# jamesdolezal/biscuit

Hardware: AMD Instinct MI355X
Metric: tiles/sec at MC-dropout=30, 299x299x3 (Xception, slide-level pred/sigma reduce) (higher is better)
Workload: dtype f16; 1 GPU; BASELINE.json config 2: 1000 synthetic 299x299x3 tiles/slide, Xception f16 storage + MFMA, fp32 accumulation / BN / MC head, MC=30, batch=256, 17664 tiles/GPU resident in HBM; f16 is the 16-bit mode that holds the 1e-3 tile/slide tolerance on O(1)-logit weights (bf16, the type config 2 names, runs 5-6 % slower and misses it: bf16_value); mc_mode=head, mc_n=30, batch=256, hip_streams=2, grids_sized_for_mask=False, parallelism=slide-sharded dp1, one all-gather of slide (pred, sigma, n)

## Files before the change

biscuit_amd/csrc/biscuit_hip.hip:

```cpp
#include "bq_ctx.h"

#include <math.h>
#include <cmath>
#include <stdlib.h>
#include <string.h>

namespace {

std::string g_create_error;

constexpr int pad16(int c) { return (c + 15) / 16 * 16; }

enum LayerFlags : int {
    F_RES = 1,
    F_DWTMP = 2,
    F_SPLIT_TMP = 4,
    F_POOLED = 8
};

struct Layer {
    const char* name;
    const char* out_name;
    int cin, cout;
    int ldi, ldo;
// ... 236 lines not shown

#define TAP_AT(name, buf, H, C, ld) \
    do { int _t = tap_nhwc(w, name, buf, H, C, ld); if (_t) return _t < 0 ? _t : BQ_OK; } while (0)
#define TAP(name, li, buf) TAP_AT(name, buf, kLayers[li].H, kLayers[li].cout, kLayers[li].ldo)

GemmParams gemm_params(const bq_ctx* c, int li, int n, const void* in, const void* residual, void* out) {
    const Layer& L = kLayers[li];
    const GemmLayer& G = c->layers[li];
    GemmParams p{};
    p.in = in; p.wp = G.wp; p.dw = G.dw; p.scale = G.scale; p.bias = G.bias; p.residual = residual; p.out = out;
    p.M = n * L.H * L.H;
    p.K = L.kpad; p.KBtot = L.kpad / (is16(c->cfg.dtype) ? 16 : 8); p.kb0 = 0; p.k_off = 0;
    p.NFp = G.nfp; p.Nstore = L.ldo; p.ldo = L.ldo; p.ldi = L.ldi;
    p.H = L.H; p.W = L.H; p.Hi = L.Hi; p.Wi = L.Hi; p.relu = L.relu;
    return p;
}

struct ConvBufs {
    const void* in; void* out;
    const void* residual = nullptr;
    void* split_tmp = nullptr;
    void* dwtmp = nullptr;
    float* gap_out = nullptr;
};

int launch_conv(const Walk& w, int li, const Route& rt, const ConvBufs& b) {
    bq_ctx* c = w.c;
    const Layer& L = kLayers[li];
    const GemmLayer& G = c->layers[li];
    if (w.plan) { w.note(L.prod == PROD_S2 ? L.out_name : L.name, route_text(rt)); return BQ_OK; }
    const int dtype = c->cfg.dtype, n = w.n, vec = is16(dtype) ? 8 : 4;
    hipStream_t s = w.s;
    const void* residual = (L.flags & F_RES) ? b.residual : nullptr;
    void* dwtmp = (L.flags & F_DWTMP) ? b.dwtmp : nullptr;
    void* split_tmp = (L.flags & F_SPLIT_TMP) ? b.split_tmp : nullptr;
    GemmParams p = gemm_params(c, li, n, b.in, residual, b.out);
    const double es = (double)esize(c);
    const double M = (double)p.M;
    const bool dwp = L.prod == PROD_DW || L.prod == PROD_DW_RELU;
    const double flops = 2.0 * M * L.cin * L.cout + (dwp ? 18.0 * M * L.cin : 0.0);
    const double in_rows = (double)n * L.Hi * L.Hi;
    const double kin = L.prod == PROD_IM2COL ? (double)L.ldi : (double)L.cin;
    const double bytes = es * (in_rows * kin * (L.prod == PROD_S2 ? 0.25 : 1.0) + M * L.cout * (residual ? 2.0 : 1.0)) +
                         es * (double)L.cin * L.cout;
    char cls[96];
    snprintf(cls, sizeof cls, "%s_k%d_n%d_%dx%d",
             L.prod == PROD_S2 ? "res1x1s2" : (L.prod == PROD_IM2COL ? "conv3x3" : "sepconv"), L.cin, L.cout, L.H, L.H);
    const bool two = rt.conv == R_DW_THEN_EXIT;
    ProfScope ps(c, s, two ? std::string("split_") + cls : std::string(cls), two ? 0.0 : flops, two ? 0.0 : bytes);
    const char* what = "launch ";
    int e = 0;
    switch (rt.conv) {
    case R_STREAM:
        what = "launch(stream) ";
        e = launch_sepconv_stream(dtype, L.kpad, L.cout, L.prod == PROD_DW_RELU, b.in, G.wp16, G.dw, G.scale, G.bias, b.out, n, L.H, L.H,
                                  L.relu, c->num_cus, s);
        break;
    case R_TILE:
        what = "launch(tile) ";
        e = launch_tile_conv(dtype, b.in, G.wp, G.scale, G.bias, b.out, n, L.H, L.H, L.Hi, L.Hi, L.relu, c->num_cus, s);
        break;
    case R_DW_THEN_EXIT: {
        const bool gap = rt.gap;
        {
            ProfScope pd(c, s, std::string("dw3x3_") + cls, 18.0 * M * L.cin, 2.0 * es * M * L.cin);
            what = "launch(dw3x3) ";
            e = launch_dw3x3(dtype, b.in, G.dw, dwtmp, n, L.H, L.H, L.ldi, L.prod == PROD_DW_RELU, s);
        }
        if (e) break;
        ProfScope pg(c, s, std::string(gap ? "gemm_gap_" : "gemm_") + cls, 2.0 * M * L.cin * L.cout + (gap ? M * L.cout : 0.0),
                     gap ? es * M * L.cin + 4.0 * n * L.cout : es * (M * L.cin + M * L.cout * (residual ? 2.0 : 1.0)));
        what = "launch(exit_gemm) ";
        e = launch_exit_gemm(dtype, dwtmp, G.wp16, G.scale, G.bias, b.out, gap ? b.gap_out : nullptr, n, L.H * L.H, L.kpad, L.cout, L.relu,
                             c->feat_mul, s);
        break;
    }
    case R_S2_TILED_GEMM:
        what = "launch(gemm_tile s2) ";
        e = launch_gemm_tile(dtype, p, s, false);
        break;
    case R_WIDE:
        what = "launch(wide) ";
        e = launch_sepconv_wide(dtype, L.prod, p, G.wp16, c->num_cus, s);
        break;
    case R_FUSED_GEMM:
        for (int sp = 0; sp < rt.nsplit && e == 0; ++sp) {
            const bool last = sp == rt.nsplit - 1;
            p.K = L.kpad / rt.nsplit;
            p.k_off = sp * p.K;
            p.kb0 = sp * (p.K / (2 * vec));
            p.bias = last ? G.bias : nullptr;
            p.relu = last ? L.relu : 0;
            p.residual = last ? (rt.nsplit > 1 ? split_tmp : residual) : (sp > 0 ? split_tmp : nullptr);
            p.out = last ? b.out : split_tmp;
            e = launch_gemm(dtype, L.prod, rt.shape, p, s);
        }
        break;
// ... 7 lines not shown
    Route rt;
    RUN(route_for(w, li, false, &rt));
    if (gap) *gap = rt.gap;
    return launch_conv(w, li, rt, b);
}

int launch_front_route(const Walk& w, const uint8_t* u8, void* out) {
    bq_ctx* c = w.c;
    const int n = w.n;
    const GemmLayer& G = c->layers[kConv2];
    if (w.plan) { w.note(kLayers[kConv2].name, kRouteNames[R_FRONT]); return BQ_OK; }
    {
        ProfScope ps(c, w.s, "stage_stats", 2.0 * n * kStaged, (double)n * kStaged);
        if (launch_stage_stats(u8, n, 299, c->d_stage_stats, w.s)) return fail(c, BQ_ERR_HIP, "stage stats launch failed");
    }
    const double p1 = (double)n * 149 * 149, p2 = (double)n * 147 * 147;
    ProfScope ps(c, w.s, "front_stage_stem_conv2", 2.0 * p1 * 27 * 32 + 2.0 * p2 * 288 * 64 + 4.0 * n * kStaged,
                 (double)n * kStaged + (double)esize(c) * p2 * 64);
    const int e = launch_front(c->cfg.dtype, u8, reinterpret_cast<const unsigned long long*>(c->d_stage_stats), c->front_ws16, c->stem_s,
                               c->stem_b, c->front_wc16, G.scale, G.bias, out, n, c->num_cus, w.s);
    return e ? launch_failed(c, "launch(front)", "", e) : BQ_OK;
}

int launch_block_end(const Walk& w, int li, const Route& rt, const void* x, const void* y, void* out) {
    bq_ctx* c = w.c;
    const Layer& L = kLayers[li];
    const GemmLayer& G = c->layers[li];
    const GemmLayer& G2 = c->layers[li - 1];
    const int dtype = c->cfg.dtype, n = w.n, ci = L.ldi, co = L.ldo;
    hipStream_t s = w.s;
    const double es = (double)esize(c), M = (double)n * L.Hi * L.Hi, Mo = (double)n * L.H * L.H;
    if (rt.kind == R_CONV_THEN_POOL) {
        RUN(launch_conv(w, li, rt, {x, out}));
        TAP(L.name, li, out);
        if (w.plan) return BQ_OK;
        char cls[64];
        snprintf(cls, sizeof cls, "maxpool_add_%d_c%d", L.Hi, L.cout);
        ProfScope ps(c, s, cls, 9.0 * Mo * co, es * ((double)n * L.Hi * L.Hi * co + 2.0 * Mo * co));
        if (launch_pool_add(y, out, out, n, L.Hi, L.Hi, co, dtype, s)) return fail(c, BQ_ERR_HIP, "pool_add launch failed");
        return BQ_OK;
    }
    if (w.plan) { w.note(L.out_name, route_text(rt)); return BQ_OK; }
    if (rt.kind == R_BLOCK_TAIL) {
        char cls[64];
        snprintf(cls, sizeof cls, "blocktail_%d_c%d", L.Hi, L.cout);
        ProfScope ps(c, s, cls, 2.0 * M * co * co + 18.0 * M * co + 2.0 * Mo * ci * co + 9.0 * Mo * co,
                     es * (M * co + Mo * ci + Mo * co) + es * ((double)co * co + (double)ci * co));
        const int e = launch_block_tail(dtype, co, co, ci, y, G2.wp16, G2.dw, G2.scale, G2.bias, x, G.wp16, G.scale, G.bias, out, n,
                                        L.Hi, L.Hi, c->num_cus, s);
        return e ? launch_failed(c, "launch(block tail) ", kLayers[li - 1].name, e) : BQ_OK;
    }
    ProfScope ps(c, s, std::string("respool_") + std::to_string(L.Hi) + "_c" + std::to_string(L.cout),
                 2.0 * Mo * L.cin * L.cout + 9.0 * Mo * co, es * ((double)n * L.Hi * L.Hi * co + Mo * co + Mo * ci) + es * (double)L.cin * L.cout);
    const int e = launch_gemm_tile(dtype, gemm_params(c, li, n, x, y, out), s, true);
    return e ? launch_failed(c, "launch(gemm_tile pool) ", L.name, e) : BQ_OK;
}

int strided_block(const Walk& w, int s1, const void* x, void* t1, void* t2, void* out) {
    RUN(run_conv(w, s1, {x, t1}));
    TAP(kLayers[s1].name, s1, t1);
    Route end;
    RUN(route_for(w, s1 + 2, false, &end));
    if (end.kind != R_BLOCK_TAIL) {
        RUN(run_conv(w, s1 + 1, {t1, t2}));
        TAP(kLayers[s1 + 1].name, s1 + 1, t2);
    }
    RUN(launch_block_end(w, s1 + 2, end, x, end.kind == R_BLOCK_TAIL ? t1 : t2, out));
    if (w.tapped()) return BQ_OK;
    TAP(kLayers[s1 + 2].out_name, s1 + 2, out);
    return BQ_OK;
}

int backbone_impl(const Walk& w, const void* in_nchw, float* feat, unsigned char* ws, const uint8_t* u8 = nullptr) {
    bq_ctx* c = w.c;
    const int n = w.n, dt = c->cfg.dtype;
    hipStream_t s = w.s;
    const WsLayout L = ws_layout(c, n, 1);
    auto at = [&](size_t off) { return reinterpret_cast<void*>(reinterpret_cast<uintptr_t>(ws) + off); };
    void* A = at(L.a); void* B = at(L.b); void* C = at(L.c); void* R = at(L.r);
    const double es = (double)esize(c);
    Route front;
    RUN(route_for(w, kConv2, u8 != nullptr, &front));
    if (front.kind == R_FRONT) {
        RUN(launch_front_route(w, u8, B));
    } else {
        if (u8) {
            in_nchw = at(L.staged);
            if (!w.plan) RUN(bq_stage(c, u8, n, at(L.staged), (bq_stream_t)s));
        }
        if (wants(w.want(), "staged")) {
// ... 8 lines not shown
            ProfScope ps(c, s, "stem_conv1_3x3s2", 2.0 * px * 27 * 32, es * ((double)n * kStaged + px * 32));
            if (launch_stem1(in_nchw, n, c->stem_w, c->stem_s, c->stem_b, A, dt, s)) return fail(c, BQ_ERR_HIP, "stem1 launch failed");
        }
        TAP_AT("block1_conv1", A, 149, 32, 32);
        RUN(launch_conv(w, kConv2, front, {A, B}));
    }
    TAP(kLayers[kConv2].name, kConv2, B);
    void* X = B; void* Y = R;
    for (int s1 = kBlock2; s1 < kBlock5; s1 += 3) {
        RUN(strided_block(w, s1, X, A, C, Y));
        if (w.tapped()) return BQ_OK;
        void* t = X; X = Y; Y = t;
    }
    void* S = B; Y = A;
    for (int s1 = kBlock5; s1 < kBlock13; s1 += 3) {
        RUN(run_conv(w, s1, {X, Y, nullptr, nullptr, S}));
        TAP(kLayers[s1].name, s1, Y);
        RUN(run_conv(w, s1 + 1, {Y, C, nullptr, nullptr, S}));
        TAP(kLayers[s1 + 1].name, s1 + 1, C);
        RUN(run_conv(w, s1 + 2, {C, Y, X, nullptr, S}));
        void* t = X; X = Y; Y = t;
        TAP(kLayers[s1 + 2].out_name, s1 + 2, X);
    }
    RUN(strided_block(w, kBlock13, X, Y, C, S));
    if (w.tapped()) return BQ_OK;
    RUN(run_conv(w, kBlock14, {S, Y, nullptr, C, X}));
    TAP(kLayers[kBlock14].name, kBlock14, Y);
    bool pooled = false;
    RUN(run_conv(w, kBlock14 + 1, {Y, C, nullptr, S, X, feat}, &pooled));
    if (!pooled) {
        TAP(kLayers[kBlock14 + 1].name, kBlock14 + 1, C);
        if (w.plan) {
            w.note("global_avg_pool", "GAP_KERNEL");
        } else {
            ProfScope ps(c, s, "global_avg_pool", (double)n * 100 * 2048, es * (double)n * 100 * 2048 + 4.0 * n * 2048);
            if (launch_gap(C, n, 100, 2048, 2048, feat, c->feat_mul, dt, s)) return fail(c, BQ_ERR_HIP, "gap launch failed");
        }
    }
    if (w.want()) return fail(c, BQ_ERR_ARG, std::string("unknown activation: ") + w.want());
    return BQ_OK;
}

int head_impl(bq_ctx* c, const float* feat, int n, int64_t tile0, int mc_n, int pass0, uint64_t seed,
              int init, int finalize, float* state, float* mean2, float* std2, unsigned char* ws,
              hipStream_t s) {
    const WsLayout L = ws_layout(c, n, mc_n);
    float* h0 = (float*)(ws + L.h0);
    float* h1 = (float*)(ws + L.h1);
    float* rmax = (float*)(ws + L.rmax);
    const unsigned thresh = c->drop_thresh;
    const float dscale = c->drop_scale;
    const int rows = n * mc_n;
// ... 218 lines not shown
            if (we->second.n < 4) return fail(c, BQ_ERR_WEIGHTS, "bad size for " + name + "/wexp");
            memcpy(&wexp, hb + (we->second.p - c->d_blob), 4);
            if (wexp < -64 || wexp > 64) return fail(c, BQ_ERR_WEIGHTS, name + "/wexp must lie in [-64, 64]");
        }
        c->head[layer] = HeadLayer{wh->second.p, wl->second.p, reinterpret_cast<const float*>(bi->second.p), K, wexp};
    }
    c->loaded = true;
    return BQ_OK;
}

int bq_stream_create_masked(bq_ctx* c, const uint32_t* cu_mask, int mask_words, bq_stream_t* out) {
    if (!c || !cu_mask || mask_words <= 0 || !out) return fail(c, BQ_ERR_ARG, "bq_stream_create_masked: bad argument");
    hipStream_t s = nullptr;
    DeviceGuard guard(c->device);
    if (!guard.ok) return fail(c, BQ_ERR_HIP, "hipSetDevice failed");
    HIPCHK(c, hipExtStreamCreateWithCUMask(&s, (uint32_t)mask_words, cu_mask));
    *out = (bq_stream_t)s;
    return BQ_OK;
}

int bq_set_option(bq_ctx* c, const char* name, int value) {
    if (!c || !name) return fail(c, BQ_ERR_ARG, "bq_set_option: bad argument");
    if (strcmp(name, "inflate_variant") == 0 && (value == 0 || value == 5)) { c->inflate_variant = value; return BQ_OK; }
    return fail(c, BQ_ERR_ARG, std::string("bq_set_option: unknown option or value: ") + name);
}

int bq_set_num_cus(bq_ctx* c, int n) {
    if (!c || n < 0 || n > 1024) return fail(c, BQ_ERR_ARG, "bq_set_num_cus: bad argument");
    int dev_cus = 256;
    if (n == 0) {
        hipDeviceProp_t prop;
        if (hipGetDeviceProperties(&prop, c->device) == hipSuccess && prop.multiProcessorCount > 0) dev_cus = prop.multiProcessorCount;
    }
    c->num_cus = n > 0 ? n : dev_cus;
    return BQ_OK;
}

int bq_stream_destroy(bq_ctx* c, bq_stream_t stream) {
    if (!c || !stream) return fail(c, BQ_ERR_ARG, "bq_stream_destroy: bad argument");
    HIPCHK(c, hipStreamDestroy((hipStream_t)stream));
    return BQ_OK;
}

int bq_backbone(bq_ctx* c, const void* d_in, int n, float* d_feat, void* d_ws, size_t ws_bytes,
                bq_stream_t stream) {
    if (!c || !d_in || !d_feat || !d_ws || n <= 0 || n > c->cfg.max_batch) return fail(c, BQ_ERR_ARG, "bq_backbone: bad argument");
// ... 128 lines not shown
```

biscuit_amd/csrc/bq_common.h:

```cpp
#pragma once
#include <hip/hip_runtime.h>
#include <stdint.h>
#include <stddef.h>


struct BqLdsAttr {
    static constexpr int kMaxDev = 64;
    size_t set[kMaxDev] = {};
    int ensure(const void* kern, size_t lds) {
        int dev = -1;
        if (hipGetDevice(&dev) != hipSuccess || dev < 0 || dev >= kMaxDev) dev = -1;
        if (dev >= 0 && lds <= set[dev]) return 0;
        const hipError_t e = hipFuncSetAttribute(kern, hipFuncAttributeMaxDynamicSharedMemorySize, (int)lds);
        if (e != hipSuccess) return (int)e;
        if (dev >= 0) set[dev] = lds;
        return 0;
    }
};

typedef __bf16 bf16_t;
typedef __bf16 bf16x8 __attribute__((ext_vector_type(8)));
typedef _Float16 f16_t;
typedef _Float16 f16x8 __attribute__((ext_vector_type(8)));
typedef float f32x16 __attribute__((ext_vector_type(16)));
// ... 35 lines not shown
    int Nstore;
    int ldo;
    int ldi;
    int H, W;
    int Hi, Wi;
    int relu;
    int unused[2];
};

size_t gemm_lds_bytes(int dtype, int shape, int K);
int launch_gemm(int dtype, int prod, int shape, const GemmParams& p, hipStream_t s);
int gemm_tile_rows(int shape);
bool wide_supported(int dtype, int prod, int nfp, int H, int W, int K, int Nstore, int ldi, int ldo, long long M, bool residual);
int launch_sepconv_wide(int dtype, int prod, const GemmParams& p, const void* wp16, int num_cus, hipStream_t s);
bool stream_supported(int dtype, int cin, int cout, bool relu_in, long long n, int H, int W);
int launch_sepconv_stream(int dtype, int cin, int cout, bool relu_in, const void* in, const void* wp16, const float* dw,
                          const float* scale, const float* bias, void* out, int n, int H, int W, int relu, int num_cus,
                          hipStream_t s);
bool tail_supported(int dtype, int cin, int cout, int cx, long long n, int H, int W);
int launch_block_tail(int dtype, int cin, int cout, int cx, const void* y1, const void* wp16, const float* dw,
                      const float* scale, const float* bias, const void* x, const void* wr16, const float* rscale,
                      const float* rbias, void* out, int n, int H, int W, int num_cus, hipStream_t s);
int launch_dw3x3(int dtype, const void* in, const float* dw, void* out, int n, int H, int W, int C, int relu, hipStream_t s);
int launch_gemm_tile(int dtype, const GemmParams& p, hipStream_t s, bool pool);
bool exit_supported(int dtype, int K, int N, int HW, long long n);
int launch_exit_gemm(int dtype, const void* in, const void* wp16, const float* scale, const float* bias, void* out, float* gap,
                     int n, int HW, int K, int N, int relu, float gap_mul, hipStream_t s);
int launch_tile_conv(int dtype, const void* in, const void* wp, const float* scale, const float* bias, void* out, int n, int H,
                     int W, int Hi, int Wi, int relu, int num_cus, hipStream_t s);

int launch_stage_stats(const uint8_t* tiles, int n, int px, double* stats_scratch, hipStream_t s);
bool front_supported(int dtype, long long n);
int launch_front(int dtype, const uint8_t* tiles, const unsigned long long* stats, const void* ws16, const float* s_scale,
                 const float* s_bias, const void* wc16, const float* c_scale, const float* c_bias, void* out, int n, int num_cus,
                 hipStream_t s);
int launch_stem1(const void* in_nchw, int n, const float* w27x32, const float* scale,
                 const float* bias, void* out_nhwc, int dtype, hipStream_t s);
int launch_pool_add(const void* y, const void* res, void* out, int n, int Hi, int Wi, int C,
                    int dtype, hipStream_t s);
int launch_gap(const void* x, int n, int HW, int C, int ld, float* feat, float mul, int dtype, hipStream_t s);
int launch_head_dense(const float* in, const void* wh, const void* wl, const float* bias, int wexp, float* out, float* rmax,
                      int rows, int K, int mc_n, int pass0, int in_row_is_tile, int layer, unsigned seed_lo, unsigned seed_hi,
                      unsigned thresh, float dscale, long long tile0, const long long* tile0_dev, const long long* tile_idx,
                      hipStream_t s);
int launch_head_final(const float* h1, int n, int mc_n, int pass0, long long tile0, const long long* tile0_dev, const long long* tile_idx,
                      unsigned seed_lo, unsigned seed_hi, unsigned thresh, float dscale,
                      const float* w2, const float* b2, int init, int finalize, float* state,
                      float* mean2, float* std2, hipStream_t s);
int launch_to_f32_nhwc(const void* x, long long rows, int C, int ld, float* out, int dtype,
                       hipStream_t s);
// ... 26 lines not shown
```

biscuit_amd/csrc/bq_ctx.h:

```cpp
#pragma once
#include "../../include/biscuit_hip.h"
#include "bq_common.h"
#include "bq_rounds.h"

#include <map>
#include <string>
#include <vector>

struct Blob { const unsigned char* p = nullptr; size_t n = 0; };

constexpr int kNumLayers = 39;

struct GemmLayer {
    const void* wp = nullptr;
    const void* wp16 = nullptr;
    const float* scale = nullptr;
    const float* bias = nullptr;
    const float* dw = nullptr;
    int nfp = 0;
};

struct HeadLayer {
    const void* wh = nullptr; const void* wl = nullptr; const float* bias = nullptr; int k = 0;
    int wexp = 0;
// ... 2 lines not shown
struct ProfRec { int cls; hipEvent_t a, b; };

struct bq_ctx {
    bq_config cfg{};
    int device = 0;
    std::string err;
    unsigned char* d_blob = nullptr;
    size_t blob_bytes = 0;
    std::map<std::string, Blob> entries;
    GemmLayer layers[kNumLayers];
    const float* stem_w = nullptr; const float* stem_s = nullptr; const float* stem_b = nullptr;
    const void* front_ws16 = nullptr;
    const void* front_wc16 = nullptr;
    const float* logits_w = nullptr; const float* logits_b = nullptr;
    HeadLayer head[2];
    unsigned drop_thresh = 0;
    float drop_scale = 1.f;
    bool loaded = false;
    int num_cus = 256;
    float* d_srgb_lut = nullptr;
    const long long* d_tile0 = nullptr;
    const long long* d_tile_idx = nullptr;
    int inflate_variant = 5;
    float feat_mul = 1.f;
    double* d_stage_stats = nullptr;
    bool prof = false;
    std::vector<std::string> prof_names;
    std::vector<double> prof_flops, prof_bytes;
    std::vector<int64_t> prof_launches;
    std::vector<double> prof_ms;
    std::vector<ProfRec> prof_recs;
    std::vector<hipEvent_t> ev_pool;
    size_t ev_used = 0;
};

#define BQ_INTERNAL __attribute__((visibility("hidden")))

BQ_INTERNAL int fail(bq_ctx* c, int code, const std::string& msg);

#define HIPCHK(c, expr)                                                                 \
    do {                                                                                \
        hipError_t _e = (hipError_t)(expr);                                             \
        if (_e != hipSuccess)                                                           \
            return fail((c), BQ_ERR_HIP, std::string(#expr) + ": " + hipGetErrorString(_e)); \
    } while (0)

// ... 50 lines not shown
```

biscuit_amd/csrc/kernels_exit.hip:

```cpp
#include "mfma16_common.h"

namespace {

constexpr int XMF = 7;
constexpr int XN = 256, XK = 64;
constexpr int XA_STR = XK * 2 + 32;
constexpr int XA_BUF = 128 * XA_STR;

template <typename T>
struct ExitParams {
    const T* in;
    const uint4* wp16;
    const float* scale;
    const float* bias;
    T* out;
    float* gap;
    int n, HW, K, N, relu;
    float gap_mul;
};

template <typename T, bool GAP>
__global__ void __launch_bounds__(256, 2) exit_gemm_kernel(const ExitParams<T> p) {
    if constexpr (H16<T>::F16) bq_f16_saturate();
    extern __shared__ __attribute__((aligned(16))) unsigned char smem[];
    const int tid = threadIdx.x, lane = tid & 63;
    const int wave = __builtin_amdgcn_readfirstlane(tid >> 6);
    const int px = lane & 15, g = lane >> 4;
    const int ntn = p.N / XN;
    const int tile = xcd_tile(blockIdx.x, gridDim.x);
    const int img = tile / ntn, nt = tile - img * ntn;
    const int NF = p.N / 16, NC = p.K / XK;
    const int n0 = nt * XN + wave * 64;

    const int jp = tid & 7;
    const T* arow[4];
#pragma unroll
    for (int q = 0; q < 4; ++q) {
        int row = (tid + q * 256) >> 3;
        row = row < p.HW ? row : p.HW - 1;
        arow[q] = p.in + ((size_t)img * p.HW + row) * p.K + jp * 8;
    }
#define XLOAD_A(c)  _Pragma("unroll") for (int q = 0; q < 4; ++q) areg[q] = *reinterpret_cast<const u32x4s*>(arow[q] + (c) * XK)
#define XSTORE_A(buf) _Pragma("unroll") for (int q = 0; q < 4; ++q) \
        *reinterpret_cast<u32x4s*>(smem + (buf) * XA_BUF + ((tid + q * 256) >> 3) * XA_STR + jp * 16) = areg[q]
// ... 47 lines not shown
#pragma unroll
    for (int q = 0; q < 2; ++q) {
        const int ch = n0 + 32 * q + 8 * g;
        const float4 s0 = *reinterpret_cast<const float4*>(p.scale + ch), s1 = *reinterpret_cast<const float4*>(p.scale + ch + 4);
        const float4 b0 = *reinterpret_cast<const float4*>(p.bias + ch), b1 = *reinterpret_cast<const float4*>(p.bias + ch + 4);
        float sum[8];
#pragma unroll
        for (int e = 0; e < 8; ++e) sum[e] = 0.f;
#pragma unroll
        for (int i = 0; i < XMF; ++i) {
            unsigned o[4];
            bn_pair4<T>(acc[i][2 * q], acc[i][2 * q + 1], s0, s1, b0, b1, o);
#pragma unroll
            for (int e = 0; e < 4; ++e) asm("v_pk_max_i16 %0, %1, %2" : "=v"(o[e]) : "v"(o[e]), "v"(lo2));
            const int row = 16 * i + px;
            if constexpr (GAP) {
                if (row < p.HW) {
#pragma unroll
                    for (int e = 0; e < 4; ++e) {
                        const f32x2s v = unpack2<T>(o[e]);
                        sum[2 * e] += v.x; sum[2 * e + 1] += v.y;
                    }
                }
            } else {
                if (row < p.HW)
                    *reinterpret_cast<uint4*>(p.out + ((size_t)img * p.HW + row) * p.N + ch) = make_uint4(o[0], o[1], o[2], o[3]);
            }
        }
        if constexpr (GAP) {
#pragma unroll
            for (int e = 0; e < 8; ++e) {
                float v = sum[e];
                v += __builtin_bit_cast(float, __builtin_amdgcn_update_dpp(0, __builtin_bit_cast(int, v), 0x111, 0xf, 0xf, true));
                v += __builtin_bit_cast(float, __builtin_amdgcn_update_dpp(0, __builtin_bit_cast(int, v), 0x112, 0xf, 0xf, true));
                v += __builtin_bit_cast(float, __builtin_amdgcn_update_dpp(0, __builtin_bit_cast(int, v), 0x114, 0xf, 0xf, true));
                v += __builtin_bit_cast(float, __builtin_amdgcn_update_dpp(0, __builtin_bit_cast(int, v), 0x118, 0xf, 0xf, true));
                sum[e] = v / (float)p.HW * p.gap_mul;
            }
            if (px == 15) {
                float* dst = p.gap + (size_t)img * p.N + ch;
                *reinterpret_cast<float4*>(dst) = make_float4(sum[0], sum[1], sum[2], sum[3]);
                *reinterpret_cast<float4*>(dst + 4) = make_float4(sum[4], sum[5], sum[6], sum[7]);
            }
        }
    }
}

template <typename T>
int launch_exit_t(const void* in, const void* wp16, const float* scale, const float* bias, void* out, float* gap, int n, int HW,
                  int K, int N, int relu, float gap_mul, hipStream_t s) {
    ExitParams<T> p{};
    p.in = reinterpret_cast<const T*>(in); p.wp16 = reinterpret_cast<const uint4*>(wp16); p.scale = scale; p.bias = bias;
    p.out = reinterpret_cast<T*>(out); p.gap = gap; p.n = n; p.HW = HW; p.K = K; p.N = N; p.relu = relu; p.gap_mul = gap_mul;
    const int grid = n * (N / XN);
    const size_t lds = 2 * XA_BUF;
    if (gap) hipLaunchKernelGGL((exit_gemm_kernel<T, true>), dim3(grid), dim3(256), lds, s, p);
    else hipLaunchKernelGGL((exit_gemm_kernel<T, false>), dim3(grid), dim3(256), lds, s, p);
    return (int)hipGetLastError();
}

}

bool exit_supported(int dtype, int K, int N, int HW, long long n) {
    return (dtype == 1 || dtype == 2) && HW > 0 && HW <= 16 * XMF && K % XK == 0 && K >= 2 * XK && N % XN == 0 &&
           n > 0 && n * (long long)(N / XN) < (1ll << 30) && n * (long long)HW * (K > N ? K : N) * 2 < (1ll << 40);
}

int launch_exit_gemm(int dtype, const void* in, const void* wp16, const float* scale, const float* bias, void* out, float* gap,
                     int n, int HW, int K, int N, int relu, float gap_mul, hipStream_t s) {
    if (!exit_supported(dtype, K, N, HW, n)) return (int)hipErrorInvalidValue;
    return dtype == 2 ? launch_exit_t<f16_t>(in, wp16, scale, bias, out, gap, n, HW, K, N, relu, gap_mul, s)
                      : launch_exit_t<bf16_t>(in, wp16, scale, bias, out, gap, n, HW, K, N, relu, gap_mul, s);
}
```

biscuit_amd/csrc/kernels_split.hip:

```cpp
#include "gemm_common.h"

namespace {
using namespace bqk;

__device__ __forceinline__ unsigned relu2s(unsigned x) { return relu_pk16(x); }

template <typename T, bool RELU>
__global__ void __launch_bounds__(256) dw3x3_kernel(const T* __restrict__ in, const float* __restrict__ dw,
                                                    T* __restrict__ out, int n, int H, int W, int C) {
    if constexpr (H16<T>::F16) bq_f16_saturate();
    const int ppp = C / 8;
    const long long gid = (long long)blockIdx.x * blockDim.x + threadIdx.x;
    if (gid >= (long long)n * W * ppp) return;
    const int piece = (int)(gid % ppp);
    const int x = (int)((gid / ppp) % W);
    const int img = (int)(gid / ((long long)ppp * W));
    float w[9][8];
#pragma unroll
    for (int t = 0; t < 9; ++t) {
        const float4 a = *reinterpret_cast<const float4*>(dw + (size_t)t * C + piece * 8);
        const float4 b = *reinterpret_cast<const float4*>(dw + (size_t)t * C + piece * 8 + 4);
        w[t][0] = a.x; w[t][1] = a.y; w[t][2] = a.z; w[t][3] = a.w;
        w[t][4] = b.x; w[t][5] = b.y; w[t][6] = b.z; w[t][7] = b.w;
    }
// ... 30 lines not shown
        for (int dx = 0; dx < 3; ++dx) {
            float f[8];
            unpack<T>(r0[dx], f);
#pragma unroll
            for (int j = 0; j < 8; ++j) acc[j] = fmaf(w[dx][j], f[j], acc[j]);
            unpack<T>(r1[dx], f);
#pragma unroll
            for (int j = 0; j < 8; ++j) acc[j] = fmaf(w[3 + dx][j], f[j], acc[j]);
            unpack<T>(r2[dx], f);
#pragma unroll
            for (int j = 0; j < 8; ++j) acc[j] = fmaf(w[6 + dx][j], f[j], acc[j]);
        }
        *reinterpret_cast<uint4*>(obase + ((size_t)y * W + x) * C) = pack<T>(acc);
#pragma unroll
        for (int k = 0; k < 3; ++k) { r0[k] = r1[k]; r1[k] = r2[k]; }
    }
}

constexpr int BM = 128, BN = 128, BK = 64;
constexpr int A_ROW = BK * 2 + 16;
constexpr int A_BUF = BM * A_ROW;
constexpr int ST_ROW = BN * 2 + 16;

enum { EPI_PLAIN = 0, EPI_POOL = 2 };

template <typename T, int PF, bool S2, int EPI = EPI_PLAIN>
__global__ void __launch_bounds__(256) gemm_tile_kernel(const GemmParams p) {
    if constexpr (H16<T>::F16) bq_f16_saturate();
    extern __shared__ __attribute__((aligned(16))) unsigned char smem[];
    const int tid = threadIdx.x, lane = tid & 63, wave = tid >> 6;
    const int wm = wave >> 1, wn = wave & 1;
    const int r32 = lane & 31, h = lane >> 5;
    const int ntn = p.NFp / 4;
    const int tile = xcd_tile(blockIdx.x, gridDim.x);
    const int mt = tile / ntn, nt = tile - mt * ntn;
    const int m0 = mt * BM;
    const int K = p.K, KB = K / 16, NC = (K + BK - 1) / BK;
    const T* __restrict__ A = reinterpret_cast<const T*>(p.in);

    const int jp = tid & 7;
    size_t arow[4];
#pragma unroll
    for (int q = 0; q < 4; ++q) {
        int row = m0 + ((tid + q * 256) >> 3);
        row = row < p.M ? row : p.M - 1;
        if constexpr (S2) {
            const int hw = p.H * p.W;
            const int img = row / hw, rem = row - img * hw;
            const int y = rem / p.W, x = rem - y * p.W;
            arow[q] = ((size_t)(img * p.Hi + 2 * y) * p.Wi + 2 * x) * p.ldi;
        } else {
            arow[q] = (size_t)row * p.ldi;
        }
    }
    auto load_a = [&](int c, uint4 (&r)[4]) {
#pragma unroll
        for (int q = 0; q < 4; ++q) {
            const int k0 = c * BK + jp * 8;
            const int kc = k0 < K ? k0 : 0;
            uint4 v = *reinterpret_cast<const uint4*>(A + arow[q] + kc);
            if (k0 >= K) v = make_uint4(0, 0, 0, 0);
            r[q] = v;
        }
    };
    auto store_a = [&](int buf, const uint4 (&r)[4]) {
#pragma unroll
        for (int q = 0; q < 4; ++q)
// ... 60 lines not shown
                sc[0] = t.x; sc[1] = t.y; sc[2] = t.z; sc[3] = t.w;
            }
            if (p.bias) {
                const float4 t = *reinterpret_cast<const float4*>(p.bias + n0);
                bi[0] = t.x; bi[1] = t.y; bi[2] = t.z; bi[3] = t.w;
            }
#pragma unroll
            for (int i = 0; i < 2; ++i) {
                const int rl = wm * 64 + i * 32 + r32;
                const int m = m0 + rl;
                float v[4];
#pragma unroll
                for (int e = 0; e < 4; ++e) v[e] = fmaf(acc[i][j][g * 4 + e], sc[e], bi[e]);
                if (res && m < p.M && n0 < p.Nstore) {
                    float rv[4];
                    load4<T>(res + (size_t)m * p.ldo + n0, rv);
#pragma unroll
                    for (int e = 0; e < 4; ++e) v[e] += rv[e];
                }
                if (p.relu) {
#pragma unroll
                    for (int e = 0; e < 4; ++e) v[e] = fmaxf(v[e], 0.f);
                }
                store4<T>(reinterpret_cast<T*>(smem + (size_t)rl * ST_ROW) + nl, v);
            }
        }
    __syncthreads();
    if constexpr (EPI == EPI_POOL) {
        const T* __restrict__ y = reinterpret_cast<const T*>(p.residual);
        T* __restrict__ out = reinterpret_cast<T*>(p.out);
        const int pc = tid & 15;
        const int ncol = nt * BN + pc * 8;
        const int pt = (p.Hi & 1) ? 1 : 0, pl = (p.Wi & 1) ? 1 : 0;
        if (ncol < p.Nstore) {
            const int hw = p.H * p.W;
            constexpr int RU = 2;
            for (int r0 = tid >> 4; r0 < BM; r0 += 16 * RU) {
                uint4 u[RU][9];
                int mrow[RU];
#pragma unroll
                for (int k = 0; k < RU; ++k) {
                    int m = m0 + r0 + 16 * k;
                    mrow[k] = m;
                    m = m < p.M ? m : p.M - 1;
                    const int img = m / hw, rem = m - img * hw;
                    const int yo = rem / p.W, xo = rem - yo * p.W;
#pragma unroll
                    for (int dy = 0; dy < 3; ++dy) {
                        int yy = 2 * yo + dy - pt;
                        yy = yy < 0 ? 0 : (yy > p.Hi - 1 ? p.Hi - 1 : yy);
#pragma unroll
                        for (int dx = 0; dx < 3; ++dx) {
                            int xx = 2 * xo + dx - pl;
                            xx = xx < 0 ? 0 : (xx > p.Wi - 1 ? p.Wi - 1 : xx);
                            u[k][dy * 3 + dx] = *reinterpret_cast<const uint4*>(y + ((size_t)(img * p.Hi + yy) * p.Wi + xx) * p.ldo + ncol);
                        }
                    }
                }
#pragma unroll
                for (int k = 0; k < RU; ++k) {
                    const int r = r0 + 16 * k;
                    if (r >= BM || mrow[k] >= p.M) continue;
                    float mx[8];
#pragma unroll
                    for (int j = 0; j < 8; ++j) mx[j] = -INFINITY;
#pragma unroll
                    for (int t = 0; t < 9; ++t) {
                        const T* e = reinterpret_cast<const T*>(&u[k][t]);
#pragma unroll
                        for (int j = 0; j < 8; ++j) mx[j] = fmaxf(mx[j], (float)e[j]);
                    }
                    const uint4 ru = *reinterpret_cast<const uint4*>(smem + (size_t)r * ST_ROW + pc * 16);
                    const T* re = reinterpret_cast<const T*>(&ru);
                    uint4 ou;
                    T* oe = reinterpret_cast<T*>(&ou);
#pragma unroll
                    for (int j = 0; j < 8; ++j) oe[j] = (T)(mx[j] + (float)re[j]);
                    *reinterpret_cast<uint4*>(out + (size_t)mrow[k] * p.ldo + ncol) = ou;
                }
            }
        }
    } else {
        unsigned char* __restrict__ out = reinterpret_cast<unsigned char*>(p.out);
        const int pc = tid & 15;
        const int ncol = nt * BN + pc * 8;
        if (ncol < p.Nstore) {
            for (int r = tid >> 4; r < BM; r += 16) {
                const int m = m0 + r;
                if (m < p.M)
                    *reinterpret_cast<uint4*>(out + ((size_t)m * p.ldo + ncol) * 2) =
                        *reinterpret_cast<const uint4*>(smem + (size_t)r * ST_ROW + pc * 16);
            }
        }
    }
}

}

namespace {
template <typename T>
int launch_dw3x3_t(const void* in, const float* dw, void* out, int n, int H, int W, int C, int relu, hipStream_t s) {
    const long long total = (long long)n * W * (C / 8);
    const int grid = (int)((total + 255) / 256);
    if (relu)
        hipLaunchKernelGGL((dw3x3_kernel<T, true>), dim3(grid), dim3(256), 0, s, (const T*)in, dw, (T*)out, n, H, W, C);
    else
        hipLaunchKernelGGL((dw3x3_kernel<T, false>), dim3(grid), dim3(256), 0, s, (const T*)in, dw, (T*)out, n, H, W, C);
    return (int)hipGetLastError();
}
}

int launch_dw3x3(int dtype, const void* in, const float* dw, void* out, int n, int H, int W, int C, int relu, hipStream_t s) {
    return dtype == 2 ? launch_dw3x3_t<f16_t>(in, dw, out, n, H, W, C, relu, s)
                      : launch_dw3x3_t<bf16_t>(in, dw, out, n, H, W, C, relu, s);
}

int launch_gemm_tile(int dtype, const GemmParams& p, hipStream_t s, bool pool) {
    if (p.NFp % 4 != 0 || p.K % 16 != 0 || (pool && !p.residual)) return (int)hipErrorInvalidValue;
    const size_t lds = 2 * A_BUF > BM * ST_ROW ? 2 * A_BUF : BM * ST_ROW;
    const int grid = ((p.M + BM - 1) / BM) * (p.NFp / 4);
    if (pool) {
        if (dtype == 2) hipLaunchKernelGGL((gemm_tile_kernel<f16_t, 4, true, EPI_POOL>), dim3(grid), dim3(256), lds, s, p);
        else hipLaunchKernelGGL((gemm_tile_kernel<bf16_t, 4, true, EPI_POOL>), dim3(grid), dim3(256), lds, s, p);
    } else {
        if (dtype == 2) hipLaunchKernelGGL((gemm_tile_kernel<f16_t, 4, true>), dim3(grid), dim3(256), lds, s, p);
        else hipLaunchKernelGGL((gemm_tile_kernel<bf16_t, 4, true>), dim3(grid), dim3(256), lds, s, p);
    }
    return (int)hipGetLastError();
}
```

Baseline: 33500 tiles/s.

## Fuse next layer's depthwise 3x3 into exit GEMM and pool-GEMM epilogues

In the exit flow (block 13 end, block 14 sepconvs), the following layer's depthwise 3x3 is computed inside the producing kernel's epilogue. The output tile for a whole image is staged into padded LDS and convolved there, so the standalone dw3x3 launch and its HBM round-trip of the intermediate are skipped. The pool-GEMM switches to one tile per image, and the exit GEMM gets a DWN variant with larger LDS. This adds LDS pressure and may lower occupancy and change grid shape, in exchange for fewer launches and less memory traffic. It is gated by an exit_fusion option that defaults on for 16-bit types.

```diff
diff --git a/biscuit_amd/csrc/biscuit_hip.hip b/biscuit_amd/csrc/biscuit_hip.hip
--- a/biscuit_amd/csrc/biscuit_hip.hip
+++ b/biscuit_amd/csrc/biscuit_hip.hip
@@ -282,7 +282,18 @@
     void* split_tmp = nullptr;
     void* dwtmp = nullptr;
     float* gap_out = nullptr;
+    int dw_next = -1;
+    bool dw_done = false;
 };
+
+bool fuses_dw(const Walk& w, int cons, const char* unwritten_a, const char* unwritten_b = nullptr) {
+    const bq_ctx* c = w.c;
+    if (!c->exit_fusion || !is16(c->cfg.dtype) || wants(w.want(), unwritten_a, unwritten_b)) return false;
+    std::string why;
+    const Layer& L = kLayers[cons];
+    return L.prod == PROD_DW && kLayers[cons - 1].H == L.H && kLayers[cons - 1].ldo == L.ldi && L.ldi == L.kpad &&
+           choose_route(c, cons, w.n, false, w.want(), &why).kind == R_DW_THEN_EXIT;
+}
 
 int launch_conv(const Walk& w, int li, const Route& rt, const ConvBufs& b) {
     bq_ctx* c = w.c;
@@ -322,17 +333,19 @@
         break;
     case R_DW_THEN_EXIT: {
         const bool gap = rt.gap;
-        {
+        if (b.dw_next >= 0 && gap) return fail(c, BQ_ERR_ARG, std::string("the pooling epilogue writes no tensor to run a depthwise on: ") + L.name);
+        if (!b.dw_done) {
             ProfScope pd(c, s, std::string("dw3x3_") + cls, 18.0 * M * L.cin, 2.0 * es * M * L.cin);
             what = "launch(dw3x3) ";
             e = launch_dw3x3(dtype, b.in, G.dw, dwtmp, n, L.H, L.H, L.ldi, L.prod == PROD_DW_RELU, s);
         }
         if (e) break;
-        ProfScope pg(c, s, std::string(gap ? "gemm_gap_" : "gemm_") + cls, 2.0 * M * L.cin * L.cout + (gap ? M * L.cout : 0.0),
+        ProfScope pg(c, s, std::string(gap ? "gemm_gap_" : "gemm_") + cls,
+                     2.0 * M * L.cin * L.cout + (gap ? M * L.cout : 0.0) + (b.dw_next >= 0 ? 18.0 * M * L.cout : 0.0),
                      gap ? es * M * L.cin + 4.0 * n * L.cout : es * (M * L.cin + M * L.cout * (residual ? 2.0 : 1.0)));
         what = "launch(exit_gemm) ";
-        e = launch_exit_gemm(dtype, dwtmp, G.wp16, G.scale, G.bias, b.out, gap ? b.gap_out : nullptr, n, L.H * L.H, L.kpad, L.cout, L.relu,
-                             c->feat_mul, s);
+        e = launch_exit_gemm(dtype, b.dw_done ? b.in : dwtmp, G.wp16, G.scale, G.bias, b.out, gap ? b.gap_out : nullptr, n, L.H * L.H,
+                             L.kpad, L.cout, L.relu, c->feat_mul, b.dw_next >= 0 ? c->layers[b.dw_next].dw : nullptr, L.H, s);
         break;
     }
     case R_S2_TILED_GEMM:
@@ -386,7 +399,7 @@
     return e ? launch_failed(c, "launch(front)", "", e) : BQ_OK;
 }
 
-int launch_block_end(const Walk& w, int li, const Route& rt, const void* x, const void* y, void* out) {
+int launch_block_end(const Walk& w, int li, const Route& rt, const void* x, const void* y, void* out, int dw_next = -1) {
     bq_ctx* c = w.c;
     const Layer& L = kLayers[li];
     const GemmLayer& G = c->layers[li];
@@ -415,12 +428,15 @@
         return e ? launch_failed(c, "launch(block tail) ", kLayers[li - 1].name, e) : BQ_OK;
     }
     ProfScope ps(c, s, std::string("respool_") + std::to_string(L.Hi) + "_c" + std::to_string(L.cout),
-                 2.0 * Mo * L.cin * L.cout + 9.0 * Mo * co, es * ((double)n * L.Hi * L.Hi * co + Mo * co + Mo * ci) + es * (double)L.cin * L.cout);
-    const int e = launch_gemm_tile(dtype, gemm_params(c, li, n, x, y, out), s, true);
+                 2.0 * Mo * L.cin * L.cout + 9.0 * Mo * co + (dw_next >= 0 ? 18.0 * Mo * co : 0.0),
+                 es * ((double)n * L.Hi * L.Hi * co + Mo * co + Mo * ci) + es * (double)L.cin * L.cout);
+    GemmParams p = gemm_params(c, li, n, x, y, out);
+    if (dw_next >= 0) p.dw = c->layers[dw_next].dw;
+    const int e = launch_gemm_tile(dtype, p, s, true, dw_next >= 0);
     return e ? launch_failed(c, "launch(gemm_tile pool) ", L.name, e) : BQ_OK;
 }
 
-int strided_block(const Walk& w, int s1, const void* x, void* t1, void* t2, void* out) {
+int strided_block(const Walk& w, int s1, const void* x, void* t1, void* t2, void* out, int dw_next = -1) {
     RUN(run_conv(w, s1, {x, t1}));
     TAP(kLayers[s1].name, s1, t1);
     Route end;
@@ -429,7 +445,8 @@
         RUN(run_conv(w, s1 + 1, {t1, t2}));
         TAP(kLayers[s1 + 1].name, s1 + 1, t2);
     }
-    RUN(launch_block_end(w, s1 + 2, end, x, end.kind == R_BLOCK_TAIL ? t1 : t2, out));
+    if (dw_next >= 0 && end.kind != R_POOL_GEMM) return fail(w.c, BQ_ERR_ARG, "only the POOL_GEMM block end runs the next layer's depthwise");
+    RUN(launch_block_end(w, s1 + 2, end, x, end.kind == R_BLOCK_TAIL ? t1 : t2, out, dw_next));
     if (w.tapped()) return BQ_OK;
     TAP(kLayers[s1 + 2].out_name, s1 + 2, out);
     return BQ_OK;
@@ -484,12 +501,23 @@
         void* t = X; X = Y; Y = t;
         TAP(kLayers[s1 + 2].out_name, s1 + 2, X);
     }
-    RUN(strided_block(w, kBlock13, X, Y, C, S));
+    Route end13;
+    RUN(route_for(w, kBlock13 + 2, false, &end13));
+    const Layer& L13 = kLayers[kBlock13 + 2];
+    const bool dw1 = end13.kind == R_POOL_GEMM && pool_dw_supported(L13.H, L13.H, n, c->layers[kBlock13 + 2].nfp) &&
+                     fuses_dw(w, kBlock14, L13.out_name, L13.name);
+    RUN(strided_block(w, kBlock13, X, Y, C, S, dw1 ? kBlock14 : -1));
     if (w.tapped()) return BQ_OK;
-    RUN(run_conv(w, kBlock14, {S, Y, nullptr, C, X}));
+    const bool dw2 = fuses_dw(w, kBlock14 + 1, kLayers[kBlock14].name);
+    ConvBufs b1{S, Y, nullptr, C, X};
+    b1.dw_done = dw1;
+    b1.dw_next = dw2 ? kBlock14 + 1 : -1;
+    RUN(run_conv(w, kBlock14, b1));
     TAP(kLayers[kBlock14].name, kBlock14, Y);
     bool pooled = false;
-    RUN(run_conv(w, kBlock14 + 1, {Y, C, nullptr, S, X, feat}, &pooled));
+    ConvBufs b2{Y, C, nullptr, S, X, feat};
+    b2.dw_done = dw2;
+    RUN(run_conv(w, kBlock14 + 1, b2, &pooled));
     if (!pooled) {
         TAP(kLayers[kBlock14 + 1].name, kBlock14 + 1, C);
         if (w.plan) {
@@ -754,6 +782,7 @@
 int bq_set_option(bq_ctx* c, const char* name, int value) {
     if (!c || !name) return fail(c, BQ_ERR_ARG, "bq_set_option: bad argument");
     if (strcmp(name, "inflate_variant") == 0 && (value == 0 || value == 5)) { c->inflate_variant = value; return BQ_OK; }
+    if (strcmp(name, "exit_fusion") == 0 && (value == 0 || value == 1)) { c->exit_fusion = value != 0; return BQ_OK; }
     return fail(c, BQ_ERR_ARG, std::string("bq_set_option: unknown option or value: ") + name);
 }
 
diff --git a/biscuit_amd/csrc/bq_common.h b/biscuit_amd/csrc/bq_common.h
--- a/biscuit_amd/csrc/bq_common.h
+++ b/biscuit_amd/csrc/bq_common.h
@@ -81,10 +81,11 @@
                       const float* scale, const float* bias, const void* x, const void* wr16, const float* rscale,
                       const float* rbias, void* out, int n, int H, int W, int num_cus, hipStream_t s);
 int launch_dw3x3(int dtype, const void* in, const float* dw, void* out, int n, int H, int W, int C, int relu, hipStream_t s);
-int launch_gemm_tile(int dtype, const GemmParams& p, hipStream_t s, bool pool);
+int launch_gemm_tile(int dtype, const GemmParams& p, hipStream_t s, bool pool, bool pool_dw = false);
+bool pool_dw_supported(int H, int W, long long n, int nfp);
 bool exit_supported(int dtype, int K, int N, int HW, long long n);
 int launch_exit_gemm(int dtype, const void* in, const void* wp16, const float* scale, const float* bias, void* out, float* gap,
-                     int n, int HW, int K, int N, int relu, float gap_mul, hipStream_t s);
+                     int n, int HW, int K, int N, int relu, float gap_mul, const float* dw_next, int W, hipStream_t s);
 int launch_tile_conv(int dtype, const void* in, const void* wp, const float* scale, const float* bias, void* out, int n, int H,
                      int W, int Hi, int Wi, int relu, int num_cus, hipStream_t s);
 
diff --git a/biscuit_amd/csrc/bq_ctx.h b/biscuit_amd/csrc/bq_ctx.h
--- a/biscuit_amd/csrc/bq_ctx.h
+++ b/biscuit_amd/csrc/bq_ctx.h
@@ -48,6 +48,7 @@
     const long long* d_tile0 = nullptr;
     const long long* d_tile_idx = nullptr;
     int inflate_variant = 5;
+    bool exit_fusion = true;
     float feat_mul = 1.f;
     double* d_stage_stats = nullptr;
     bool prof = false;
diff --git a/biscuit_amd/csrc/kernels_exit.hip b/biscuit_amd/csrc/kernels_exit.hip
--- a/biscuit_amd/csrc/kernels_exit.hip
+++ b/biscuit_amd/csrc/kernels_exit.hip
@@ -6,6 +6,7 @@
 constexpr int XN = 256, XK = 64;
 constexpr int XA_STR = XK * 2 + 32;
 constexpr int XA_BUF = 128 * XA_STR;
+constexpr int XT_STR = XN * 2 + 16;
 
 template <typename T>
 struct ExitParams {
@@ -17,9 +18,11 @@
     float* gap;
     int n, HW, K, N, relu;
     float gap_mul;
+    const float* dwn;
+    int W;
 };
 
-template <typename T, bool GAP>
+template <typename T, bool GAP, bool DWN = false>
 __global__ void __launch_bounds__(256, 2) exit_gemm_kernel(const ExitParams<T> p) {
     if constexpr (H16<T>::F16) bq_f16_saturate();
     extern __shared__ __attribute__((aligned(16))) unsigned char smem[];
@@ -113,6 +116,11 @@
                         sum[2 * e] += v.x; sum[2 * e + 1] += v.y;
                     }
                 }
+            } else if constexpr (DWN) {
+                if (row < p.HW) {
+                    const int cell = row + 2 * (row / p.W) + p.W + 3;
+                    *reinterpret_cast<uint4*>(smem + cell * XT_STR + (ch - nt * XN) * 2) = make_uint4(o[0], o[1], o[2], o[3]);
+                }
             } else {
                 if (row < p.HW)
                     *reinterpret_cast<uint4*>(p.out + ((size_t)img * p.HW + row) * p.N + ch) = make_uint4(o[0], o[1], o[2], o[3]);
@@ -135,16 +143,68 @@
             }
         }
     }
+    if constexpr (DWN) {
+        const int pc = tid & 31;
+        const int W = p.W, H = p.HW / W, WP = W + 2;
+        for (int b = tid >> 5; b < 2 * (W + 3) + 2 * (H - 1); b += 8) {
+            const int k = b - (W + 3);
+            const int cell = k < 0 ? b : (k < 2 * (H - 1) ? (1 + (k >> 1)) * WP + W + 1 + (k & 1) : H * WP + W + 1 + (k - 2 * (H - 1)));
+            *reinterpret_cast<uint4*>(smem + cell * XT_STR + pc * 16) = make_uint4(0, 0, 0, 0);
+        }
+        __syncthreads();
+        const float* const dwp = p.dwn + nt * XN + pc * 8;
+        float w[9][8];
+#pragma unroll
+        for (int t = 0; t < 9; ++t) {
+            const float4 a = *reinterpret_cast<const float4*>(dwp + (size_t)t * p.N);
+            const float4 b = *reinterpret_cast<const float4*>(dwp + (size_t)t * p.N + 4);
+            w[t][0] = a.x; w[t][1] = a.y; w[t][2] = a.z; w[t][3] = a.w;
+            w[t][4] = b.x; w[t][5] = b.y; w[t][6] = b.z; w[t][7] = b.w;
+        }
+        T* const obase = p.out + (size_t)img * p.HW * p.N + nt * XN + pc * 8;
+        int y = (tid >> 5) / W, x = (tid >> 5) - y * W;
+        for (int pix = tid >> 5; pix < p.HW; pix += 8) {
+            const unsigned char* const tp = smem + (y * WP + x) * XT_STR + pc * 16;
+            float acc[8];
+#pragma unroll
+            for (int j = 0; j < 8; ++j) acc[j] = 0.f;
+#pragma unroll
+            for (int dx = 0; dx < 3; ++dx) {
+#pragma unroll
+                for (int dy = 0; dy < 3; ++dy) {
+                    const uint4 v = *reinterpret_cast<const uint4*>(tp + (dy * WP + dx) * XT_STR);
+                    const unsigned u[4] = {v.x, v.y, v.z, v.w};
+#pragma unroll
+                    for (int e = 0; e < 4; ++e) {
+                        acc[2 * e] = H16<T>::fma_lo(u[e], w[dy * 3 + dx][2 * e], acc[2 * e]);
+                        acc[2 * e + 1] = H16<T>::fma_hi(u[e], w[dy * 3 + dx][2 * e + 1], acc[2 * e + 1]);
+                    }
+                }
+            }
+            *reinterpret_cast<uint4*>(obase + (size_t)pix * p.N) = pack<T>(acc);
+            x += 8;
+            while (x >= W) { x -= W; ++y; }
+        }
+    }
 }
 
 template <typename T>
 int launch_exit_t(const void* in, const void* wp16, const float* scale, const float* bias, void* out, float* gap, int n, int HW,
-                  int K, int N, int relu, float gap_mul, hipStream_t s) {
+                  int K, int N, int relu, float gap_mul, const float* dw_next, int W, hipStream_t s) {
     ExitParams<T> p{};
     p.in = reinterpret_cast<const T*>(in); p.wp16 = reinterpret_cast<const uint4*>(wp16); p.scale = scale; p.bias = bias;
     p.out = reinterpret_cast<T*>(out); p.gap = gap; p.n = n; p.HW = HW; p.K = K; p.N = N; p.relu = relu; p.gap_mul = gap_mul;
+    p.dwn = dw_next; p.W = W;
     const int grid = n * (N / XN);
     const size_t lds = 2 * XA_BUF;
+    if (dw_next) {
+        const size_t tile = (size_t)(HW / W + 2) * (W + 2) * XT_STR, lds_t = tile > lds ? tile : lds;
+        if (lds_t > 80 * 1024) return (int)hipErrorInvalidValue;
+        static BqLdsAttr attr;
+        if (const int e = attr.ensure(reinterpret_cast<const void*>(&exit_gemm_kernel<T, false, true>), lds_t)) return e;
+        hipLaunchKernelGGL((exit_gemm_kernel<T, false, true>), dim3(grid), dim3(256), lds_t, s, p);
+        return (int)hipGetLastError();
+    }
     if (gap) hipLaunchKernelGGL((exit_gemm_kernel<T, true>), dim3(grid), dim3(256), lds, s, p);
     else hipLaunchKernelGGL((exit_gemm_kernel<T, false>), dim3(grid), dim3(256), lds, s, p);
     return (int)hipGetLastError();
@@ -158,8 +218,9 @@
 }
 
 int launch_exit_gemm(int dtype, const void* in, const void* wp16, const float* scale, const float* bias, void* out, float* gap,
-                     int n, int HW, int K, int N, int relu, float gap_mul, hipStream_t s) {
+                     int n, int HW, int K, int N, int relu, float gap_mul, const float* dw_next, int W, hipStream_t s) {
     if (!exit_supported(dtype, K, N, HW, n)) return (int)hipErrorInvalidValue;
-    return dtype == 2 ? launch_exit_t<f16_t>(in, wp16, scale, bias, out, gap, n, HW, K, N, relu, gap_mul, s)
-                      : launch_exit_t<bf16_t>(in, wp16, scale, bias, out, gap, n, HW, K, N, relu, gap_mul, s);
-}
+    if (dw_next && (gap || W <= 0 || HW % W != 0)) return (int)hipErrorInvalidValue;
+    return dtype == 2 ? launch_exit_t<f16_t>(in, wp16, scale, bias, out, gap, n, HW, K, N, relu, gap_mul, dw_next, W, s)
+                      : launch_exit_t<bf16_t>(in, wp16, scale, bias, out, gap, n, HW, K, N, relu, gap_mul, dw_next, W, s);
+}
diff --git a/biscuit_amd/csrc/kernels_split.hip b/biscuit_amd/csrc/kernels_split.hip
--- a/biscuit_amd/csrc/kernels_split.hip
+++ b/biscuit_amd/csrc/kernels_split.hip
@@ -76,7 +76,7 @@
 constexpr int A_BUF = BM * A_ROW;
 constexpr int ST_ROW = BN * 2 + 16;
 
-enum { EPI_PLAIN = 0, EPI_POOL = 2 };
+enum { EPI_PLAIN = 0, EPI_POOL = 2, EPI_POOL_DW = 3 };
 
 template <typename T, int PF, bool S2, int EPI = EPI_PLAIN>
 __global__ void __launch_bounds__(256) gemm_tile_kernel(const GemmParams p) {
@@ -88,7 +88,9 @@
     const int ntn = p.NFp / 4;
     const int tile = xcd_tile(blockIdx.x, gridDim.x);
     const int mt = tile / ntn, nt = tile - mt * ntn;
-    const int m0 = mt * BM;
+    constexpr bool IMG = EPI == EPI_POOL_DW;
+    const int mreal = IMG ? p.H * p.W : BM;
+    const int m0 = mt * mreal;
     const int K = p.K, KB = K / 16, NC = (K + BK - 1) / BK;
     const T* __restrict__ A = reinterpret_cast<const T*>(p.in);
 
@@ -96,7 +98,8 @@
     size_t arow[4];
 #pragma unroll
     for (int q = 0; q < 4; ++q) {
-        int row = m0 + ((tid + q * 256) >> 3);
+        int row = (tid + q * 256) >> 3;
+        row = m0 + (row < mreal ? row : mreal - 1);
         row = row < p.M ? row : p.M - 1;
         if constexpr (S2) {
             const int hw = p.H * p.W;
@@ -203,11 +206,24 @@
 #pragma unroll
                     for (int e = 0; e < 4; ++e) v[e] = fmaxf(v[e], 0.f);
                 }
-                store4<T>(reinterpret_cast<T*>(smem + (size_t)rl * ST_ROW) + nl, v);
-            }
-        }
+                if constexpr (IMG) {
+                    if (rl < mreal) store4<T>(reinterpret_cast<T*>(smem + (size_t)(rl + 2 * (rl / p.W) + p.W + 3) * ST_ROW) + nl, v);
+                } else {
+                    store4<T>(reinterpret_cast<T*>(smem + (size_t)rl * ST_ROW) + nl, v);
+                }
+            }
+        }
+    if constexpr (IMG) {
+        const int WP = p.W + 2;
+        for (int b = tid >> 4; b < 2 * (p.W + 3) + 2 * (p.H - 1); b += 16) {
+            const int k = b - (p.W + 3);
+            const int cell = k < 0 ? b : (k < 2 * (p.H - 1) ? (1 + (k >> 1)) * WP + p.W + 1 + (k & 1)
+                                                            : p.H * WP + p.W + 1 + (k - 2 * (p.H - 1)));
+            *reinterpret_cast<uint4*>(smem + (size_t)cell * ST_ROW + (tid & 15) * 16) = make_uint4(0, 0, 0, 0);
+        }
+    }
     __syncthreads();
-    if constexpr (EPI == EPI_POOL) {
+    if constexpr (EPI == EPI_POOL || EPI == EPI_POOL_DW) {
         const T* __restrict__ y = reinterpret_cast<const T*>(p.residual);
         T* __restrict__ out = reinterpret_cast<T*>(p.out);
         const int pc = tid & 15;
@@ -218,14 +234,18 @@
             constexpr int RU = 2;
             for (int r0 = tid >> 4; r0 < BM; r0 += 16 * RU) {
                 uint4 u[RU][9];
-                int mrow[RU];
+                int mrow[RU], yo_[RU];
 #pragma unroll
                 for (int k = 0; k < RU; ++k) {
                     int m = m0 + r0 + 16 * k;
                     mrow[k] = m;
+                    if constexpr (IMG) {
+                        if (r0 + 16 * k >= mreal) { mrow[k] = p.M; m = m0 + mreal - 1; }
+                    }
                     m = m < p.M ? m : p.M - 1;
                     const int img = m / hw, rem = m - img * hw;
                     const int yo = rem / p.W, xo = rem - yo * p.W;
+                    yo_[k] = yo;
 #pragma unroll
                     for (int dy = 0; dy < 3; ++dy) {
                         int yy = 2 * yo + dy - pt;
@@ -251,13 +271,51 @@
 #pragma unroll
                         for (int j = 0; j < 8; ++j) mx[j] = fmaxf(mx[j], (float)e[j]);
                     }
-                    const uint4 ru = *reinterpret_cast<const uint4*>(smem + (size_t)r * ST_ROW + pc * 16);
+                    const int cell = IMG ? r + 2 * yo_[k] + p.W + 3 : r;
+                    const uint4 ru = *reinterpret_cast<const uint4*>(smem + (size_t)cell * ST_ROW + pc * 16);
                     const T* re = reinterpret_cast<const T*>(&ru);
                     uint4 ou;
                     T* oe = reinterpret_cast<T*>(&ou);
 #pragma unroll
                     for (int j = 0; j < 8; ++j) oe[j] = (T)(mx[j] + (float)re[j]);
-                    *reinterpret_cast<uint4*>(out + (size_t)mrow[k] * p.ldo + ncol) = ou;
+                    if constexpr (IMG) *reinterpret_cast<uint4*>(smem + (size_t)cell * ST_ROW + pc * 16) = ou;
+                    else *reinterpret_cast<uint4*>(out + (size_t)mrow[k] * p.ldo + ncol) = ou;
+                }
+            }
+        }
+        if constexpr (IMG) {
+            __syncthreads();
+            const int q4 = tid & 31;
+            const int ncol4 = nt * BN + q4 * 4;
+            if (ncol4 < p.Nstore) {
+                float w[9][4];
+#pragma unroll
+                for (int t = 0; t < 9; ++t) {
+                    const float4 a = *reinterpret_cast<const float4*>(p.dw + (size_t)t * p.ldo + ncol4);
+                    w[t][0] = a.x; w[t][1] = a.y; w[t][2] = a.z; w[t][3] = a.w;
+                }
+                const int WP = p.W + 2;
+                int py = (tid >> 5) / p.W, px = (tid >> 5) - py * p.W;
+                for (int pix = tid >> 5; pix < mreal; pix += 8) {
+                    const unsigned char* const tp = smem + (size_t)(py * WP + px) * ST_ROW + q4 * 8;
+                    float acc[8];
+#pragma unroll
+                    for (int j = 0; j < 8; ++j) acc[j] = 0.f;
+#pragma unroll
+                    for (int dx = 0; dx < 3; ++dx) {
+#pragma unroll
+                        for (int dy = 0; dy < 3; ++dy) {
+                            const uint2 v = *reinterpret_cast<const uint2*>(tp + (size_t)(dy * WP + dx) * ST_ROW);
+                            acc[0] = H16<T>::fma_lo(v.x, w[dy * 3 + dx][0], acc[0]);
+                            acc[1] = H16<T>::fma_hi(v.x, w[dy * 3 + dx][1], acc[1]);
+                            acc[2] = H16<T>::fma_lo(v.y, w[dy * 3 + dx][2], acc[2]);
+                            acc[3] = H16<T>::fma_hi(v.y, w[dy * 3 + dx][3], acc[3]);
+                        }
+                    }
+                    const uint4 o = pack<T>(acc);
+                    *reinterpret_cast<uint2*>(out + ((size_t)m0 + pix) * p.ldo + ncol4) = make_uint2(o.x, o.y);
+                    px += 8;
+                    while (px >= p.W) { px -= p.W; ++py; }
                 }
             }
         }
@@ -296,9 +354,22 @@
                       : launch_dw3x3_t<bf16_t>(in, dw, out, n, H, W, C, relu, s);
 }
 
-int launch_gemm_tile(int dtype, const GemmParams& p, hipStream_t s, bool pool) {
+bool pool_dw_supported(int H, int W, long long n, int nfp) {
+    return H > 0 && W > 0 && H * W <= BM && (H + 2) * (W + 2) * ST_ROW <= 48 * 1024 && n > 0 && n * (long long)(nfp / 4) < (1ll << 30);
+}
+
+int launch_gemm_tile(int dtype, const GemmParams& p, hipStream_t s, bool pool, bool pool_dw) {
     if (p.NFp % 4 != 0 || p.K % 16 != 0 || (pool && !p.residual)) return (int)hipErrorInvalidValue;
     const size_t lds = 2 * A_BUF > BM * ST_ROW ? 2 * A_BUF : BM * ST_ROW;
+    if (pool_dw) {
+        const size_t tile = (size_t)(p.H + 2) * (p.W + 2) * ST_ROW, lds_img = tile > lds ? tile : lds;
+        if (!pool || !p.dw || p.M % (p.H * p.W) != 0 || !pool_dw_supported(p.H, p.W, p.M / (p.H * p.W), p.NFp))
+            return (int)hipErrorInvalidValue;
+        const int grid_img = (p.M / (p.H * p.W)) * (p.NFp / 4);
+        if (dtype == 2) hipLaunchKernelGGL((gemm_tile_kernel<f16_t, 4, true, EPI_POOL_DW>), dim3(grid_img), dim3(256), lds_img, s, p);
+        else hipLaunchKernelGGL((gemm_tile_kernel<bf16_t, 4, true, EPI_POOL_DW>), dim3(grid_img), dim3(256), lds_img, s, p);
+        return (int)hipGetLastError();
+    }
     const int grid = ((p.M + BM - 1) / BM) * (p.NFp / 4);
     if (pool) {
         if (dtype == 2) hipLaunchKernelGGL((gemm_tile_kernel<f16_t, 4, true, EPI_POOL>), dim3(grid), dim3(256), lds, s, p);
```

New measurement: 33690 tiles/s, median of 6. About the same (+0.6%).
